# amoussawi/recoder

Hardware: AMD Instinct MI355X
Metric: train_users_per_sec (higher is better)
Workload: dtype f32 (decoder GEMMs: split 16-bit operands, f32 accumulate); 1 GPU; C2 ML-20M-like synthetic CSR 116677x20108 (lognormal degree mean 73, Zipf(1) items, values 1.0, seed 0); DynamicAutoencoder hidden=[200] tanh noise 0.5, MSE, dense Adam lr 1e-3 wd 2e-5, negative sampling; api=Recoder.train, batch_size_per_gpu=500, global_batch=500, parallelism=dp1, graph_replay=True, steps_per_graph=8, pretouch=parameters + Adam moments read 8 x in front of the clock (cache + clock warm)

## Files before the change

### recoder_amd/csrc/common.h

```cpp
#pragma once
#include <hip/hip_runtime.h>
#include <stdint.h>
#include <stdio.h>

#include "../../include/recoder_hip.h"
#include "../../include/recoder_hip_probe.h"
#include "internal.h"
int rk_tune_get(int knob);

void rk_set_error(const char *fmt, ...);

#define RK_LAUNCH(kernel, grid, block, shmem, stream, ...) \
  hipLaunchKernelGGL(kernel, grid, block, shmem, stream, __VA_ARGS__)

#define RK_CHECK_LAUNCH(name)                                              \
  do {                                                                     \
    hipError_t e__ = hipGetLastError();                                    \
    if (e__ != hipSuccess) {                                               \
      rk_set_error("%s: %s", name, hipGetErrorString(e__));                \
      return -1;                                                           \
    }                                                                      \
  } while (0)

#define RK_REQUIRE(cond, msg)                                              \
  do {                                                                     \
    if (!(cond)) {                                                         \
      rk_set_error("%s: %s", __func__, msg);                               \
      return -2;                                                           \
    }                                                                      \
  } while (0)

static inline int rk_cdiv(int64_t a, int64_t b) { return (int)((a + b - 1) / b); }

struct rk_enc_split_t;
int rk_ae_encode_fwd_at(const rk_block_t *blk, int32_t row_off, int32_t B, const float *W_en,
                        const float *b_en, int32_t h, const uint8_t *keep, float p, uint64_t seed,
                        const int64_t *cursor, int32_t cursor_off, const int64_t *users, int32_t act,
                        float *Z0, void *zt_planes, void *stream, const rk_enc_split_t *es,
                        uint64_t rng_step);
const rk_replay_t *rk_replay_get(void);
int rk_splitk_reduce(const float *ws, int M, int N, const int32_t *Kdev, int splits, const float *Zact,
                     int act, float *out, void *stream);
int rk_dz_splits(int B);
extern "C" int32_t rk_gemm_plain_bf16(void);
extern "C" int32_t rk_dw_pairs(void);
extern "C" int32_t rk_dw_encode_bwd_fused_ok(int32_t row_off, int32_t B);
int rk_adam_multi_at(const rk_adam_job_t *jobs, int32_t n_jobs, float *loss_part, int32_t n_part,
                     float denom, float *loss_out, const int64_t *cursor, int32_t cursor_off,
                     const void *table, int32_t tab_stride, const int32_t *tab_slots,
                     int64_t *cursor_next, int32_t advance, void *stream);

struct rk_small_gemm_t {
  const float *A; int lda, amode;
  const float *B; int ldb, bmode;
  int M, N, K;
  float *C; int ldc;
  const float *bias;
  int act, accumulate;
  const float *dact_y;
  int dact;
};
bool rk_small_gemm_fits(int M, int N, int K);
int rk_small_gemm(const rk_small_gemm_t *g, void *stream);
int rk_small_gemm_pair(const rk_small_gemm_t *g1, const rk_small_gemm_t *g2, void *stream);
int rk_small_gemm_pair_colsum(const rk_small_gemm_t *g1, const rk_small_gemm_t *g2, const float *cs_X,
                              int cs_rows, int cs_cols, float *cs_out, void *stream);
int rk_act_grad_colsum(float *dY, const float *Y, int rows, int cols, int act, float *db, void *stream);

__device__ __forceinline__ float rk_act(float x, int act) {
  switch (act) {
    case RK_ACT_TANH: return tanhf(x);
    case RK_ACT_SIGMOID: return 1.0f / (1.0f + expf(-x));
    case RK_ACT_RELU: return x > 0.f ? x : 0.f;
    case RK_ACT_SELU: {
      const float a = 1.6732632423543772848170429916717f;
      const float s = 1.0507009873554804934193349852946f;
      return s * (x > 0.f ? x : a * (expf(x) - 1.0f));
    }
    case RK_ACT_ELU: return x > 0.f ? x : (expf(x) - 1.0f);
    default: return x;
  }
}

__device__ __forceinline__ float rk_act_dy(float y, int act) {
  switch (act) {
    case RK_ACT_TANH: return 1.0f - y * y;
    case RK_ACT_SIGMOID: return (1.0f - y) * y;
    case RK_ACT_RELU: return y > 0.f ? 1.0f : 0.f;
    case RK_ACT_SELU: {
      const float a = 1.6732632423543772848170429916717f;
      const float s = 1.0507009873554804934193349852946f;
      return y > 0.f ? s : (y + s * a);
    }
    case RK_ACT_ELU: return y > 0.f ? 1.0f : (y + 1.0f);
    default: return 1.0f;
  }
}

__device__ __forceinline__ uint64_t rk_mix64(uint64_t z) {
  z = (z ^ (z >> 30)) * 0xbf58476d1ce4e5b9ULL;
  z = (z ^ (z >> 27)) * 0x94d049bb133111ebULL;
  return z ^ (z >> 31);
}
__device__ __forceinline__ bool rk_keep_draw(uint64_t seed, uint64_t step, uint64_t a,
                                             uint64_t b, float p) {
  uint64_t z = rk_mix64(seed + 0x9e3779b97f4a7c15ULL * (step + 1));
  z = rk_mix64(z ^ (a * 0xd1342543de82ef95ULL + b + 0x632be59bd9b4e019ULL));
  float u = (float)(z >> 40) * (1.0f / 16777216.0f);
  return u >= p;
}

struct rk_cur_t {
  const int64_t *cursor;
  int32_t off;
};
__device__ __forceinline__ int64_t rk_cur_global(const rk_cur_t &c) { return c.cursor[0] + c.off; }
__device__ __forceinline__ int64_t rk_cur_local(const rk_cur_t &c) {
  return c.cursor[0] - c.cursor[1] + c.off;
}
__device__ __forceinline__ int32_t rk_cur_stamp(const rk_cur_t &c) {
  return (int32_t)(rk_cur_global(c) & 0x3fffffff) + 1;
}

typedef __bf16 rk_bf16x2 __attribute__((ext_vector_type(2)));
typedef float rk_f32x2 __attribute__((ext_vector_type(2)));
__device__ __forceinline__ void rk_split_bf16_pair(float a, float b, uint32_t &h, uint32_t &m,
                                                   uint32_t &l) {
  const rk_f32x2 x = {a, b};
  const rk_bf16x2 hh = __builtin_convertvector(x, rk_bf16x2);
  const rk_f32x2 r1 = x - __builtin_convertvector(hh, rk_f32x2);
  const rk_bf16x2 mm = __builtin_convertvector(r1, rk_bf16x2);
  const rk_f32x2 r2 = r1 - __builtin_convertvector(mm, rk_f32x2);
  const rk_bf16x2 ll = __builtin_convertvector(r2, rk_bf16x2);
  h = __builtin_bit_cast(uint32_t, hh);
  m = __builtin_bit_cast(uint32_t, mm);
  l = __builtin_bit_cast(uint32_t, ll);
}

__device__ __forceinline__ float rk_wave_sum(float v) {
#pragma unroll
  for (int off = 32; off > 0; off >>= 1) v += __shfl_down(v, off, 64);
  return v;
}
__device__ __forceinline__ float rk_wave_max(float v) {
#pragma unroll
  for (int off = 32; off > 0; off >>= 1) v = fmaxf(v, __shfl_down(v, off, 64));
  return v;
}

__device__ __forceinline__ int rk_entry_index(const rk_block_t &b, int row, int c, uint32_t word) {
  return b.indptr[row] + b.pref_rc[(int64_t)row * b.ldw_rc + (c >> 5)] +
         __popc(word & ((1u << (c & 31)) - 1u));
}

__device__ __forceinline__ int rk_find_col(const int32_t *cols, int beg, int end, int c) {
  int lo = beg, hi = end;
  while (lo < hi) {
    int mid = (lo + hi) >> 1;
    if (cols[mid] < c) lo = mid + 1; else hi = mid;
  }
  return (lo < end && cols[lo] == c) ? lo : -1;
}
```

### recoder_amd/csrc/encoder.hip

```cpp
#include "common.h"
#include "encoder_bwd.h"
#include "planes.h"

namespace {

constexpr int FW = 8;
unsigned long long *g_enc_probe = nullptr;
#define ESTAMP(k) do { if (probe && threadIdx.x == 0) probe[(size_t)(blockIdx.x - n_split) * 8 + (k)] = wall_clock64(); } while (0)
template <int HV, int UB>
__global__ __launch_bounds__(FW * 64) void ae_encode_fwd_kernel(
    rk_block_t b, int row_off, int B, const float *__restrict__ W, const float *__restrict__ bias,
    int h, const uint8_t *__restrict__ keep, float p, float scale, uint64_t seed,
    uint64_t rng_step, const int64_t *__restrict__ users, const float *__restrict__ user_norm,
    int act, float *__restrict__ Z0, uint16_t *__restrict__ planes, int64_t plane_stride,
    int cols_pad, rk_cur_t cur, rkp::SplitW sw, int n_split, char *__restrict__ zimg, int z_kt,
    int zt_pairs, unsigned long long *probe, int z_ones) {
  __shared__ float red[FW];
  constexpr int PART_B = (FW - 1) * HV * 256 * 4;
  __shared__ __attribute__((aligned(16))) char sm_raw[PART_B > rkp::SPLIT_W_LDS ? PART_B : rkp::SPLIT_W_LDS];
  if ((int)blockIdx.x < n_split) {
    rkp::split_w_job<FW * 64>(sw, (int)blockIdx.x, sm_raw);
    return;
  }
  if (cur.cursor) {
    rng_step = (uint64_t)(rk_cur_global(cur) + 1);
    if (users) users += rk_cur_local(cur) * B;
  }
  float (*part)[HV * 256] = reinterpret_cast<float (*)[HV * 256]>(sm_raw);
  const int r = (int)blockIdx.x - n_split;
  if (r >= B) {
    if (planes) {
      for (int n = threadIdx.x; n < h; n += FW * 64) {
        const int64_t o = ((int64_t)(r >> 3) * cols_pad + n) * 8 + (r & 7);
        planes[o] = 0; planes[o + plane_stride] = 0; planes[o + 2 * plane_stride] = 0;
      }
    }
    return;
  }
  const int row = row_off + r;
  const int tid = threadIdx.x, lane = tid & 63, wid = tid >> 6;
  ESTAMP(0);
  const int beg = b.indptr[row], end = b.indptr[row + 1];
  const int n = end - beg;
  const bool implicit = b.implicit != 0;
  const int64_t uid = users ? users[row] : (int64_t)row;

  const int q = (n + FW - 1) / FW;
  const int wbeg = beg + wid * q;
  const int wend = min(end, wbeg + q);
  int item0 = 0;
  float v0 = 0.f;
  if (wbeg + lane < wend) {
    item0 = b.gcols ? b.gcols[wbeg + lane] : b.items[b.cols[wbeg + lane]];
    v0 = implicit ? 1.0f : b.vals[wbeg + lane];
  }

  float nrm;
  if (user_norm) {
    nrm = fmaxf(user_norm[uid], 1e-12f);
  } else if (implicit) {
    nrm = fmaxf(sqrtf((float)n), 1e-12f);
  } else {
    float ss = 0.f;
    for (int j = beg + tid; j < end; j += FW * 64) {
      const float v = b.vals[j];
      ss += v * v;
    }
    ss = rk_wave_sum(ss);
    if (lane == 0) red[wid] = ss;
    __syncthreads();
    float tot = 0.f;
#pragma unroll
    for (int w = 0; w < FW; ++w) tot += red[w];
    nrm = fmaxf(sqrtf(tot), 1e-12f);
  }

  if (probe) { if (item0 == 0x7fffffff && v0 == 1e30f) return; ESTAMP(1); }
  float4 acc[HV];
#pragma unroll
  for (int k = 0; k < HV; ++k) acc[k] = make_float4(0.f, 0.f, 0.f, 0.f);
  float4 bb[HV];
#pragma unroll
  for (int v = 0; v < HV; ++v) {
    const int hh = (v * 64 + lane) * 4;
    bb[v] = (bias && wid == 0 && hh < h) ? *reinterpret_cast<const float4 *>(bias + hh)
                                         : make_float4(0.f, 0.f, 0.f, 0.f);
  }

  for (int base = wbeg; base < wend; base += 64) {
    const int j = base + lane;
    int item = item0;
    float val = v0;
    if (base != wbeg && j < wend) {
      item = b.gcols ? b.gcols[j] : b.items[b.cols[j]];
      val = implicit ? 1.0f : b.vals[j];
    }
    float s = 0.f;
    if (j < wend) {
      const float xh = val / nrm;
      bool kp = true;
      if (p > 0.f) kp = keep ? (keep[j] != 0) : rk_keep_draw(seed, rng_step, (uint64_t)uid, (uint64_t)item, p);
      s = (p > 0.f) ? (kp ? xh * scale : 0.f) : xh;
      b.svals[j] = s;
    } else {
      item = 0;
    }
    unsigned long long live = __ballot(s != 0.f);
    while (live) {
      int it[UB];
      float sv[UB];
#pragma unroll
      for (int u = 0; u < UB; ++u) {
        const bool has = live != 0ull;
        const int kk = has ? __builtin_ctzll(live) : 0;
        live &= live - 1ull;
        it[u] = has ? __builtin_amdgcn_readlane(item, kk) : 0;
        sv[u] = has ? __int_as_float(__builtin_amdgcn_readlane(__float_as_int(s), kk)) : 0.f;
      }
#pragma unroll
      for (int v = 0; v < HV; ++v) {
        const int hh = min((v * 64 + lane) * 4, h - 4);
        float4 w4[UB];
#pragma unroll
        for (int u = 0; u < UB; ++u)
          w4[u] = *reinterpret_cast<const float4 *>(W + (int64_t)it[u] * h + hh);
#pragma unroll
        for (int u = 0; u < UB; ++u) {
          acc[v].x = fmaf(sv[u], w4[u].x, acc[v].x);
          acc[v].y = fmaf(sv[u], w4[u].y, acc[v].y);
          acc[v].z = fmaf(sv[u], w4[u].z, acc[v].z);
          acc[v].w = fmaf(sv[u], w4[u].w, acc[v].w);
        }
      }
    }
  }
  if (probe) { if (acc[0].x == 1.2345e30f) return; ESTAMP(2); }
  if (wid > 0) {
#pragma unroll
    for (int v = 0; v < HV; ++v)
      *reinterpret_cast<float4 *>(&part[wid - 1][(v * 64 + lane) * 4]) = acc[v];
  }
  __syncthreads();
  if (wid == 0) {
#pragma unroll
    for (int v = 0; v < HV; ++v) {
      const int hh = (v * 64 + lane) * 4;
      if (hh < h) {
        float4 a = acc[v];
        for (int w = 0; w < FW - 1; ++w) {
          const float4 o = *reinterpret_cast<const float4 *>(&part[w][hh]);
          a.x += o.x; a.y += o.y; a.z += o.z; a.w += o.w;
        }
        float4 y;
        y.x = rk_act(a.x + bb[v].x, act);
        y.y = rk_act(a.y + bb[v].y, act);
        y.z = rk_act(a.z + bb[v].z, act);
        y.w = rk_act(a.w + bb[v].w, act);
        *reinterpret_cast<float4 *>(Z0 + (int64_t)r * h + hh) = y;
        if (zimg) {
          const float sz = sw.plain ? 1.0f : rkp::SCALE_Z;
          rkp::store_split4(zimg + (int64_t)r * z_kt * rkp::LINE, hh, y, sz, sw.plain != 0);
          if (r == 0 && tid == 0) sw.scales[0] = sz;
          if ((h & 31) != 0 && hh == h - 4)
            rkp::store_split4(zimg + (int64_t)r * z_kt * rkp::LINE, h, make_float4(z_ones ? 1.f : 0.f, 0.f, 0.f, 0.f), sz,
                              sw.plain != 0);
        }
        if (planes) {
          uint32_t hp[2], mp[2], lp[2];
          if (zt_pairs) {
            uint2 hh2, ll2;
            rkp::split4(y, rkp::SCALE_Z, hh2, ll2);
            hp[0] = hh2.x; hp[1] = hh2.y; mp[0] = ll2.x; mp[1] = ll2.y; lp[0] = lp[1] = 0u;
          } else {
          rk_split_bf16_pair(y.x, y.y, hp[0], mp[0], lp[0]);
          rk_split_bf16_pair(y.z, y.w, hp[1], mp[1], lp[1]);
          }
#pragma unroll
          for (int e = 0; e < 4; ++e) {
            const int64_t o = ((int64_t)(r >> 3) * cols_pad + hh + e) * 8 + (r & 7);
            const int sh = (e & 1) * 16;
            planes[o] = (uint16_t)(hp[e >> 1] >> sh);
            planes[o + plane_stride] = (uint16_t)(mp[e >> 1] >> sh);
            planes[o + 2 * plane_stride] = (uint16_t)(lp[e >> 1] >> sh);
          }
        }
      }
    }
  }
  ESTAMP(3);
}

template <int HV>
__global__ __launch_bounds__(256) void ae_encode_bwd_kernel(
    rk_block_t b, int row_off, int B, const float *__restrict__ dZ, int h,
    float *__restrict__ G, int accumulate, float *__restrict__ gb, int n_gb) {
  ae_encode_bwd_body<HV>(b, row_off, B, dZ, h, G, accumulate, gb, n_gb, (int)blockIdx.x);
}

template <int HV, int WW>
__global__ __launch_bounds__(256) __attribute__((amdgpu_waves_per_eu(6))) void ae_encode_bwd_cols_light_kernel(
    rk_block_t b, int row_off, int B, const float *__restrict__ dZ, int h,
    float *__restrict__ G, int accumulate, float *__restrict__ gb, int n_gb) {
  ae_encode_bwd_cols_body<HV, false, WW, 2>(b, row_off, B, dZ, h, G, accumulate, gb, n_gb, (int)blockIdx.x);
}

template <int HV, int WW = 1, int U = 8>
__global__ __launch_bounds__(256) void ae_encode_bwd_cols_kernel(
    rk_block_t b, int row_off, int B, const float *__restrict__ dZ, int h,
    float *__restrict__ G, int accumulate, float *__restrict__ gb, int n_gb) {
  ae_encode_bwd_cols_body<HV, false, WW, U>(b, row_off, B, dZ, h, G, accumulate, gb, n_gb, (int)blockIdx.x);
}

}

static int encode_fwd_launch(const rk_block_t *blk, int32_t row_off, int32_t B, const float *W_en,
                             const float *b_en, int32_t h, const uint8_t *keep, float p,
                             uint64_t seed, uint64_t rng_step, const int64_t *users,
                             const float *user_norm, int32_t act, float *Z0, void *stream_,
                             void *zt_planes = nullptr, rk_cur_t cur = {nullptr, 0},
                             const rk_enc_split_t *es = nullptr, int zt_pairs = 0) {
  hipStream_t stream = (hipStream_t)stream_;
  RK_REQUIRE(h > 0 && h % 4 == 0 && h <= 1024, "h must be a multiple of 4, <= 1024");
  RK_REQUIRE(p >= 0.f && p < 1.f, "noise_prob must be in [0,1)");
  RK_REQUIRE(row_off >= 0 && B >= 0 && row_off + B <= blk->S_cap, "row slice out of range");
  RK_REQUIRE(user_norm == nullptr || users != nullptr, "user_norm is indexed by users[]");
  if (B == 0) return 0;
  const float scale = 1.0f / (float)(1.0 - (double)p);
  const int hv = rk_cdiv(h, 256);
  const int rows = zt_planes ? rk_dw3_rows_pad(B) : B;
  const int cols_pad = rk_dw3_cols_pad(h);
  const int64_t plane_stride = (int64_t)rk_dw3_rows_pad(B) * cols_pad;
  rkp::SplitW sw = {};
  int n_split = 0, z_kt = 0, z_ones = 0;
  char *zimg = nullptr;
  if (es) {
    sw = es->sw; n_split = es->n_split; zimg = es->zimg; z_kt = es->z_kt;
    z_ones = (es->z_ones && zimg && h % 32 != 0) ? 1 : 0;
  }
#define LAUNCH(HV)                                                                         \
  RK_LAUNCH((ae_encode_fwd_kernel<HV, 8>), dim3(n_split + rows), dim3(FW * 64), 0, stream, *blk, row_off, \
                     B, W_en, b_en, h, keep, p, scale, seed, rng_step, users, user_norm, act, Z0, \
                     (uint16_t *)zt_planes, plane_stride, cols_pad, cur, sw, n_split, zimg, z_kt, zt_pairs, g_enc_probe, z_ones)
  if (hv == 1) LAUNCH(1); else if (hv == 2) LAUNCH(2); else LAUNCH(4);
#undef LAUNCH
  RK_CHECK_LAUNCH("ae_encode_fwd");
  return 0;
}

extern "C" void rk_enc_probe(unsigned long long *buffer) { g_enc_probe = buffer; }

extern "C" int rk_ae_encode_fwd(const rk_block_t *blk, int32_t row_off, int32_t B,
                                const float *W_en, const float *b_en, int32_t h,
                                const uint8_t *keep, float p, uint64_t seed, uint64_t rng_step,
                                const int64_t *users, int32_t act, float *Z0, void *stream_) {
  RK_REQUIRE(b_en != nullptr, "b_en is required");
  if (const rk_replay_t *rp = rk_replay_get()) {
    const rk_cur_t cur = {rp->cursor, rp->off};
    return encode_fwd_launch(blk, row_off, B, W_en, b_en, h, keep, p, seed, 0, rp->users_base, nullptr,
                             act, Z0, stream_, nullptr, cur);
  }
  return encode_fwd_launch(blk, row_off, B, W_en, b_en, h, keep, p, seed, rng_step, users, nullptr,
                           act, Z0, stream_);
}

extern "C" int rk_ae_encode_fwd_split_w(const rk_block_t *blk, int32_t row_off, int32_t B,
                                        const float *W_en, const float *b_en, int32_t h,
                                        const uint8_t *keep, float p, uint64_t seed, uint64_t rng_step,
                                        const int64_t *users, int32_t act, float *Z0, const float *W_de,
                                        const int32_t *ranges, const rk_planes_t *pl, void *stream_) {
  RK_REQUIRE(b_en != nullptr, "b_en is required");
  RK_REQUIRE(pl && pl->h == h && blk->n_cap <= pl->n_cap, "planes were laid out for another shape");
  RK_REQUIRE((((uintptr_t)W_de) & 15) == 0, "W_de must be 16-byte aligned");
  rk_enc_split_t es = {};
  es.sw = rk_split_w_args(W_de, blk, ranges, pl);
  es.n_split = rk_cdiv(blk->n_cap, 32);
  es.zimg = nullptr;
  es.z_kt = rkp::kp_of(h) / 32;
  if (const rk_replay_t *rp = rk_replay_get()) {
    const rk_cur_t cur = {rp->cursor, rp->off};
    return encode_fwd_launch(blk, row_off, B, W_en, b_en, h, keep, p, seed, 0, rp->users_base, nullptr,
                             act, Z0, stream_, nullptr, cur, &es);
  }
  return encode_fwd_launch(blk, row_off, B, W_en, b_en, h, keep, p, seed, rng_step, users, nullptr,
                           act, Z0, stream_, nullptr, {nullptr, 0}, &es);
}

extern "C" int rk_ae_encode_fwd_planes(const rk_block_t *blk, int32_t row_off, int32_t B,
                                       const float *W_en, const float *b_en, int32_t h,
                                       const uint8_t *keep, float p, uint64_t seed, uint64_t rng_step,
                                       const int64_t *users, int32_t act, float *Z0, void *zt_planes,
                                       void *stream_) {
  RK_REQUIRE(b_en != nullptr, "b_en is required");
  RK_REQUIRE(zt_planes != nullptr && (((uintptr_t)zt_planes) & 15) == 0, "zt_planes: 16-byte aligned");
  return encode_fwd_launch(blk, row_off, B, W_en, b_en, h, keep, p, seed, rng_step, users, nullptr,
                           act, Z0, stream_, zt_planes);
}

int rk_ae_encode_fwd_at(const rk_block_t *blk, int32_t row_off, int32_t B, const float *W_en,
                        const float *b_en, int32_t h, const uint8_t *keep, float p, uint64_t seed,
                        const int64_t *cursor, int32_t cursor_off, const int64_t *users, int32_t act,
                        float *Z0, void *zt_planes, void *stream_, const rk_enc_split_t *es,
                        uint64_t rng_step) {
  const rk_cur_t cur = {cursor, cursor_off};
  return encode_fwd_launch(blk, row_off, B, W_en, b_en, h, keep, p, seed, rng_step, users, nullptr, act,
                           Z0, stream_, zt_planes, cur, es, zt_planes != nullptr && rk_dw_pairs() ? 1 : 0);
}

extern "C" int rk_ae_encode_fwd_partial(const rk_block_t *blk, int32_t row_off, int32_t B,
                                        const float *W_en, int32_t h, const uint8_t *keep, float p,
                                        uint64_t seed, uint64_t rng_step, const int64_t *users,
                                        const float *user_norm, float *Zpart, void *stream_) {
// ... 58 lines not shown
```

### recoder_amd/csrc/encoder_bwd.h

```cpp
#ifndef RK_ENCODER_BWD_H
#define RK_ENCODER_BWD_H
#include "common.h"

namespace {

template <int HV, bool DYN = false>
__device__ __forceinline__ void ae_encode_bwd_body(
    const rk_block_t &b, int row_off, int B, const float *__restrict__ dZ, int h,
    float *__restrict__ G, int accumulate, float *__restrict__ gb, int n_gb, int bid,
    int n_seg = 1, int64_t seg_stride = 0, char *sm = nullptr) {
  float (*part)[HV * 256];
  if constexpr (DYN) {
    part = reinterpret_cast<float (*)[HV * 256]>(sm);
  } else {
    __shared__ __attribute__((aligned(16))) float part_s[3][HV * 256];
    part = part_s;
  }
  const int lane = threadIdx.x & 63, wid = threadIdx.x >> 6;
  if (bid < n_gb) {
    const int gseg = bid % n_seg, j0 = (bid / n_seg) * 64 + (lane & 15) * 4;
    const int srows = ((B + n_seg - 1) / n_seg + 63) & ~63;
    const int r_lo = gseg * srows, r_hi = min(B, r_lo + srows);
    const int jj = min(j0, h - 4);
    float4 a = make_float4(0.f, 0.f, 0.f, 0.f);
    int r = r_lo + wid * 4 + (lane >> 4);
    for (; r + 7 * 16 < r_hi; r += 8 * 16) {
      float4 v[8];
#pragma unroll
      for (int u = 0; u < 8; ++u) v[u] = *reinterpret_cast<const float4 *>(dZ + (int64_t)(r + u * 16) * h + jj);
#pragma unroll
      for (int u = 0; u < 8; ++u) { a.x += v[u].x; a.y += v[u].y; a.z += v[u].z; a.w += v[u].w; }
    }
    for (; r < r_hi; r += 16) {
      const float4 v = *reinterpret_cast<const float4 *>(dZ + (int64_t)r * h + jj);
      a.x += v.x; a.y += v.y; a.z += v.z; a.w += v.w;
    }
#pragma unroll
    for (int off = 16; off <= 32; off <<= 1) {
      a.x += __shfl_xor(a.x, off, 64); a.y += __shfl_xor(a.y, off, 64);
      a.z += __shfl_xor(a.z, off, 64); a.w += __shfl_xor(a.w, off, 64);
    }
    if (lane < 16) *reinterpret_cast<float4 *>(&part[0][wid * 64 + lane * 4]) = a;
    __syncthreads();
    if (wid == 0 && lane < 16 && j0 < h) {
      float4 o = a;
      for (int w = 1; w < 4; ++w) {
        const float4 q = *reinterpret_cast<const float4 *>(&part[0][w * 64 + lane * 4]);
        o.x += q.x; o.y += q.y; o.z += q.z; o.w += q.w;
      }
      *reinterpret_cast<float4 *>(gb + gseg * h + j0) = o;
    }
    return;
  }
  const int n_b = b.counts[0];
  const int c = (bid - n_gb) / n_seg, seg = (bid - n_gb) % n_seg;
  if (c >= n_b) return;
  const uint32_t *colbits = b.bits_cr + (int64_t)c * b.ldw_cr;
  float4 acc[HV];
#pragma unroll
  for (int k = 0; k < HV; ++k) acc[k] = make_float4(0.f, 0.f, 0.f, 0.f);

  const int seg_rows = ((B + n_seg - 1) / n_seg + 63) & ~63;
  const int rbeg = row_off + seg * seg_rows;
  const int rend = min(row_off + B, rbeg + seg_rows);
  G += seg * seg_stride;
  for (int r0 = (rbeg & ~63) + wid * 64; r0 < rend; r0 += 256) {
    const int row = r0 + lane;
    bool on = false;
    float s = 0.f;
    if (row >= rbeg && row < rend) {
      on = (colbits[row >> 5] >> (row & 31)) & 1u;
      if (on) {
        const uint32_t word = b.bits_rc[(int64_t)row * b.ldw_rc + (c >> 5)];
        s = b.svals[rk_entry_index(b, row, c, word)];
      }
    }
    unsigned long long mask = __ballot(on && s != 0.f);
    while (mask) {
      int kk[8];
      float sv[8];
#pragma unroll
      for (int u = 0; u < 8; ++u) {
        const bool have = mask != 0ull;
        const int k = have ? __builtin_ctzll(mask) : 0;
        mask = have ? (mask & (mask - 1)) : 0ull;
        kk[u] = have ? (r0 + k - row_off) : 0;
        sv[u] = have ? __shfl(s, k, 64) : 0.f;
      }
#pragma unroll
      for (int v = 0; v < HV; ++v) {
        const int hh = min((v * 64 + lane) * 4, h - 4);
        float4 d4[8];
#pragma unroll
        for (int u = 0; u < 8; ++u)
          d4[u] = *reinterpret_cast<const float4 *>(dZ + (int64_t)kk[u] * h + hh);
#pragma unroll
        for (int u = 0; u < 8; ++u) {
          acc[v].x = fmaf(sv[u], d4[u].x, acc[v].x);
          acc[v].y = fmaf(sv[u], d4[u].y, acc[v].y);
          acc[v].z = fmaf(sv[u], d4[u].z, acc[v].z);
          acc[v].w = fmaf(sv[u], d4[u].w, acc[v].w);
        }
      }
    }
  }
  if (wid > 0) {
#pragma unroll
    for (int v = 0; v < HV; ++v)
      *reinterpret_cast<float4 *>(&part[wid - 1][(v * 64 + lane) * 4]) = acc[v];
  }
  __syncthreads();
  if (wid == 0) {
    float *grow = G + (int64_t)c * h;
#pragma unroll
    for (int v = 0; v < HV; ++v) {
      const int hh = (v * 64 + lane) * 4;
      if (hh < h) {
        float4 a = acc[v];
        for (int w = 0; w < 3; ++w) {
          const float4 o = *reinterpret_cast<const float4 *>(&part[w][hh]);
          a.x += o.x; a.y += o.y; a.z += o.z; a.w += o.w;
        }
        if (accumulate) {
          const float4 o = *reinterpret_cast<const float4 *>(grow + hh);
          a.x += o.x; a.y += o.y; a.z += o.z; a.w += o.w;
        }
        *reinterpret_cast<float4 *>(grow + hh) = a;
      }
    }
  }
}

template <int HV, bool DYN = false, int WW = 1, int U = 8>
__device__ __forceinline__ void ae_encode_bwd_cols_body(
    const rk_block_t &b, int row_off, int B, const float *__restrict__ dZ, int h,
    float *__restrict__ G, int accumulate, float *__restrict__ gb, int n_gb, const int bid,
    char *sm = nullptr) {
  static_assert(WW == 1 || !DYN, "the two-word window exists in the stand-alone kernel only");
  if (bid < n_gb) {
    ae_encode_bwd_body<HV, DYN>(b, row_off, B, dZ, h, G, accumulate, gb, n_gb, bid, 1, 0, sm);
    return;
  }
  float (*part)[HV * 256];
  uint16_t (*rows_l)[64];
  uint16_t *rows_h;
  int *heavy_l;
  if constexpr (DYN) {
    part = reinterpret_cast<float (*)[HV * 256]>(sm);
    rows_l = reinterpret_cast<uint16_t (*)[64]>(sm + 3 * HV * 256 * 4);
    rows_h = reinterpret_cast<uint16_t *>(sm + 3 * HV * 256 * 4 + 4 * 64 * 2);
    heavy_l = reinterpret_cast<int *>(sm + 3 * HV * 256 * 4 + 4 * 64 * 2 + (2048 + 64) * 2);
  } else {
    __shared__ __attribute__((aligned(16))) float part_s[3][HV * 256];
    __shared__ uint16_t rows_l_s[4][64];
    __shared__ uint16_t rows_h_s[WW * 2048 + 64];
    __shared__ int heavy_l_s[4];
    part = part_s; rows_l = rows_l_s; rows_h = rows_h_s; heavy_l = heavy_l_s;
  }
  const int lane = threadIdx.x & 63, wid = threadIdx.x >> 6;
  const int n_b = b.counts[0];
  const int Q = (n_b + 3) >> 2;
  const int c0 = bid - n_gb;
  if (c0 >= Q) return;
  const int c = c0 + wid * Q;
  const bool live = c < n_b;
  const int w0 = row_off >> 5, rend = row_off + B;
  const int nw = ((rend + 31) >> 5) - w0;
  uint32_t mw[WW];
  int off_w[WW];
  int total = 0;
#pragma unroll
  for (int j = 0; j < WW; ++j) {
    const int wj = lane + 64 * j;
    uint32_t m = 0;
    if (live && wj < nw) {
      m = b.bits_cr[(int64_t)c * b.ldw_cr + w0 + wj];
      const int base = (w0 + wj) << 5;
      if (base < row_off) m &= ~0u << (row_off - base);
      if (base + 32 > rend) m &= (1u << (rend - base)) - 1u;
    }
    mw[j] = m;
  }
#pragma unroll
  for (int j = 0; j < WW; ++j) {
    const int cnt = __popc(mw[j]);
    int incl = cnt;
#pragma unroll
    for (int d = 1; d < 64; d <<= 1) {
      const int t = __shfl_up(incl, d, 64);
      if (lane >= d) incl += t;
    }
    off_w[j] = total + incl - cnt;
    total += __shfl(incl, 63, 64);
  }
  const bool heavy = total > 64;
  if (lane == 0) heavy_l[wid] = heavy ? total : 0;
  if (!heavy) {
#pragma unroll
    for (int j = 0; j < WW; ++j) {
      uint32_t m = mw[j];
      int o = off_w[j];
      while (m) {
        const int k = __builtin_ctz(m);
        m &= m - 1;
        rows_l[wid][o++] = (uint16_t)(((w0 + lane + 64 * j) << 5) + k - row_off);
      }
    }
  }
  __syncthreads();
  float4 acc[HV];
#pragma unroll
  for (int k = 0; k < HV; ++k) acc[k] = make_float4(0.f, 0.f, 0.f, 0.f);
  if (live && !heavy && total > 0) {
    int row = row_off;
    float sv = 0.f;
    if (lane < total) {
      row = row_off + rows_l[wid][lane];
      const uint32_t word = b.bits_rc[(int64_t)row * b.ldw_rc + (c >> 5)];
      sv = b.svals[rk_entry_index(b, row, c, word)];
    }
    unsigned long long lv = __ballot(sv != 0.f);
    while (lv) {
      int kk[U];
      float s8[U];
#pragma unroll
      for (int u = 0; u < U; ++u) {
        const bool has = lv != 0ull;
        const int k = has ? __builtin_ctzll(lv) : 0;
        lv &= lv - 1ull;
        kk[u] = has ? __builtin_amdgcn_readlane(row, k) - row_off : 0;
        s8[u] = has ? __int_as_float(__builtin_amdgcn_readlane(__float_as_int(sv), k)) : 0.f;
      }
#pragma unroll
      for (int v = 0; v < HV; ++v) {
        const int hh = min((v * 64 + lane) * 4, h - 4);
        float4 d4[U];
#pragma unroll
        for (int u = 0; u < U; ++u)
          d4[u] = *reinterpret_cast<const float4 *>(dZ + (int64_t)kk[u] * h + hh);
#pragma unroll
        for (int u = 0; u < U; ++u) {
          acc[v].x = fmaf(s8[u], d4[u].x, acc[v].x);
          acc[v].y = fmaf(s8[u], d4[u].y, acc[v].y);
          acc[v].z = fmaf(s8[u], d4[u].z, acc[v].z);
          acc[v].w = fmaf(s8[u], d4[u].w, acc[v].w);
        }
      }
    }
  }
  if (live && !heavy && !(accumulate && total == 0)) {
    float *grow = G + (int64_t)c * h;
#pragma unroll
    for (int v = 0; v < HV; ++v) {
      const int hh = (v * 64 + lane) * 4;
      if (hh < h) {
        float4 a = acc[v];
        if (accumulate) {
          const float4 o = *reinterpret_cast<const float4 *>(grow + hh);
          a.x += o.x; a.y += o.y; a.z += o.z; a.w += o.w;
        }
        *reinterpret_cast<float4 *>(grow + hh) = a;
      }
    }
  }
  for (int j = 0; j < 4; ++j) {
    const int tot_j = heavy_l[j];
    if (tot_j == 0) continue;
    const int cj = c0 + j * Q;
    if (wid == j) {
#pragma unroll
      for (int jw = 0; jw < WW; ++jw) {
        uint32_t m = mw[jw];
        int o = off_w[jw];
        while (m) {
          const int k = __builtin_ctz(m);
          m &= m - 1;
          rows_h[o++] = (uint16_t)(((w0 + lane + 64 * jw) << 5) + k - row_off);
        }
      }
    }
    __syncthreads();
#pragma unroll
    for (int k = 0; k < HV; ++k) acc[k] = make_float4(0.f, 0.f, 0.f, 0.f);
    const int per = (tot_j + 3) >> 2;
    const int e1 = min(tot_j, (wid + 1) * per);
    for (int e0 = wid * per; e0 < e1; e0 += 64) {
      const int ne = min(64, e1 - e0);
      int row = row_off;
      float sv = 0.f;
      if (lane < ne) {
        row = row_off + rows_h[e0 + lane];
        const uint32_t word = b.bits_rc[(int64_t)row * b.ldw_rc + (cj >> 5)];
        sv = b.svals[rk_entry_index(b, row, cj, word)];
      }
      constexpr int UH = U >= 8 ? 16 : 2 * U;
      unsigned long long lv = __ballot(sv != 0.f);
      while (lv) {
        int kk[UH];
        float s16[UH];
#pragma unroll
        for (int u = 0; u < UH; ++u) {
          const bool has = lv != 0ull;
          const int k = has ? __builtin_ctzll(lv) : 0;
          lv &= lv - 1ull;
          kk[u] = has ? __builtin_amdgcn_readlane(row, k) - row_off : 0;
          s16[u] = has ? __int_as_float(__builtin_amdgcn_readlane(__float_as_int(sv), k)) : 0.f;
        }
#pragma unroll
        for (int v = 0; v < HV; ++v) {
          const int hh = min((v * 64 + lane) * 4, h - 4);
          float4 d4[UH];
#pragma unroll
          for (int u = 0; u < UH; ++u)
            d4[u] = *reinterpret_cast<const float4 *>(dZ + (int64_t)kk[u] * h + hh);
#pragma unroll
          for (int u = 0; u < UH; ++u) {
            acc[v].x = fmaf(s16[u], d4[u].x, acc[v].x);
            acc[v].y = fmaf(s16[u], d4[u].y, acc[v].y);
            acc[v].z = fmaf(s16[u], d4[u].z, acc[v].z);
            acc[v].w = fmaf(s16[u], d4[u].w, acc[v].w);
          }
        }
      }
    }
    if (wid > 0) {
#pragma unroll
      for (int v = 0; v < HV; ++v)
        *reinterpret_cast<float4 *>(&part[wid - 1][(v * 64 + lane) * 4]) = acc[v];
    }
    __syncthreads();
    if (wid == 0) {
      float *grow = G + (int64_t)cj * h;
#pragma unroll
      for (int v = 0; v < HV; ++v) {
        const int hh = (v * 64 + lane) * 4;
        if (hh < h) {
          float4 a = acc[v];
          for (int w = 0; w < 3; ++w) {
            const float4 o = *reinterpret_cast<const float4 *>(&part[w][hh]);
            a.x += o.x; a.y += o.y; a.z += o.z; a.w += o.w;
          }
          if (accumulate) {
            const float4 o = *reinterpret_cast<const float4 *>(grow + hh);
            a.x += o.x; a.y += o.y; a.z += o.z; a.w += o.w;
          }
          *reinterpret_cast<float4 *>(grow + hh) = a;
        }
      }
    }
    __syncthreads();
  }
}

}
#endif
```

### recoder_amd/csrc/fdecode.hip

```cpp
#include <stdlib.h>

#include <algorithm>

#include <type_traits>

#include "common.h"
#include "pgemm_epi.h"
#include "planes.h"

namespace {

using pg::f16x8;
using pg::f32x16;

struct FdecP {
  const char *zimg, *wimg;
  const float *scales;
  int KT;
  int M;
  const int32_t *Ndev;
  int z_rows, w_rows;
  rk_block_t blk;
  int row_off;
  float confidence, inv_B;
// ... 61 lines not shown
    words[i] = b.bits_rc[(int64_t)mrow * b.ldw_rc + min((n0 >> 5) + 2 * hf + i, b.ldw_rc - 1)];
  if (tid < 128) misc[tid] = p.bias[p.bidx[min(n0 + tid, N - 1)]];

  pg::Opnd ow = {p.wimg, (int64_t)KT * 128, KT, p.w_rows};
  pg::Stager<128, false, 8> sw;
  sw.init(ow, n0, 0, min(N, p.w_rows), wave, lane);
#pragma unroll
  for (int kt = 0; kt < KTM; ++kt) sw.issue(Wst + kt * WB, wave);
  asm volatile("" ::: "memory");
  pg::u32x4 zraw[KTM][4];
  {
    const int zlim = min(M, p.z_rows) - 1;
#pragma unroll
    for (int i = 0; i < 4; ++i) {
      const int zr = min(m0 + 32 * pr + 8 * i + (lane >> 3), zlim);
      const char *zsrc = p.zimg + (int64_t)zr * (KTM * 128) + 16 * (lane & 7);
#pragma unroll
      for (int kt = 0; kt < KTM; ++kt) zraw[kt][i] = *reinterpret_cast<const pg::u32x4 *>(zsrc + kt * 128);
    }
  }
  asm volatile("s_waitcnt vmcnt(%0) lgkmcnt(0)" ::"n"(4 * KTM) : "memory");
  __builtin_amdgcn_s_barrier();
  asm volatile("" ::: "memory");

  f32x16 acc[2];
#pragma unroll
  for (int i = 0; i < 2; ++i)
#pragma unroll
    for (int r = 0; r < 16; ++r) acc[i][r] = 0.f;
  pg::FragKC fr;
  fr.init(lane);
  char *zb = Zb + wave * 4096;
#pragma unroll
  for (int kt = 0; kt < KTM; ++kt) {
    const char *SW = Wst + kt * WB + hf * 8192;
    __builtin_amdgcn_wave_barrier();
#pragma unroll
    for (int i = 0; i < 4; ++i) {
      const int r = 8 * i + (lane >> 3);
      *reinterpret_cast<pg::u32x4 *>(zb + r * 128 + (((lane & 7) ^ pg::kc_sw(r)) << 4)) = zraw[kt][i];
    }
    __builtin_amdgcn_fence(__ATOMIC_RELEASE, "wavefront");
    __builtin_amdgcn_wave_barrier();
    __builtin_amdgcn_fence(__ATOMIC_ACQUIRE, "wavefront");
    f16x8 zh[2], zl[2];
#pragma unroll
    for (int ks = 0; ks < 2; ++ks) { zh[ks] = fr.load(zb, 0, ks, 0); if (!PLAIN) zl[ks] = fr.load(zb, 0, ks, 1); }
#pragma unroll
    for (int ks = 0; ks < 2; ++ks) {
      f16x8 wh[2], wl[2];
#pragma unroll
      for (int i = 0; i < 2; ++i) { wh[i] = fr.load(SW, i, ks, 0); if (!PLAIN) wl[i] = fr.load(SW, i, ks, 1); }
      if constexpr (PLAIN) {
#pragma unroll
        for (int i = 0; i < 2; ++i)
          acc[i] = __builtin_amdgcn_mfma_f32_32x32x16_bf16(__builtin_bit_cast(pg::bf16x8, wh[i]),
                                                           __builtin_bit_cast(pg::bf16x8, zh[ks]), acc[i], 0, 0, 0);
        continue;
      }
#pragma unroll
      for (int i = 0; i < 2; ++i) acc[i] = __builtin_amdgcn_mfma_f32_32x32x16_f16(wh[i], zl[ks], acc[i], 0, 0, 0);
#pragma unroll
      for (int i = 0; i < 2; ++i) acc[i] = __builtin_amdgcn_mfma_f32_32x32x16_f16(wl[i], zh[ks], acc[i], 0, 0, 0);
#pragma unroll
      for (int i = 0; i < 2; ++i) acc[i] = __builtin_amdgcn_mfma_f32_32x32x16_f16(wh[i], zh[ks], acc[i], 0, 0, 0);
    }
  }

  const float inv = 1.0f / (p.scales[0] * p.scales[1]);
  const bool implicit = b.implicit != 0;
  const int nh = n0 + 64 * hf;
  float lsum = 0.f, gmax = 0.f;
  auto loss_pass = [&](auto implicit_c) {
    constexpr bool IMPL = decltype(implicit_c)::value;
#pragma unroll
    for (int i = 0; i < 2; ++i) {
      const uint32_t w = words[i];
#pragma unroll
      for (int r = 0; r < 16; ++r) {
        const int nl = (r & 3) + 8 * (r >> 2) + 4 * lh;
        const int n = nh + 32 * i + nl;
        const bool ok = (m < M) && (n < N);
        const float o = acc[i][r] * inv + misc[64 * hf + 32 * i + nl];
        float tv = 0.f;
        if (ok && ((w >> nl) & 1u)) {
          tv = 1.0f;
          if (!IMPL) tv = b.vals[rk_entry_index(b, mrow, n, w)];
        }
        float l, g;
        if (LOSS == pg::LOSS_MSE) {
          const float wgt = (tv > 0.f) ? (1.0f + p.confidence) : 1.0f;
          const float d = o - tv;
          l = wgt * (d * d);
          g = (2.0f * d) * (wgt * p.inv_B);
        } else {
          const float ls = fminf(o, 0.f) - log1pf(expf(-fabsf(o)));
          l = (1.0f - tv) * o - ls;
          const float sg = 1.0f / (1.0f + expf(-o));
          g = (sg - tv) * p.inv_B;
        }
        if (ok) { lsum += l; gmax = fmaxf(gmax, fabsf(g)); } else g = 0.f;
        acc[i][r] = g;
      }
    }
  };
  auto loss_pass_mse_implicit = [&]() {
    const float c = p.confidence, inv_B2 = 2.0f * p.inv_B;
#pragma unroll
    for (int i = 0; i < 2; ++i) {
      const int nrem = N - (nh + 32 * i);
      uint32_t vmask = nrem >= 32 ? 0xffffffffu : (nrem <= 0 ? 0u : ((1u << nrem) - 1u));
      if (m >= M) vmask = 0u;
      const uint32_t vsh = vmask >> (4 * lh), wsh = (words[i] & vmask) >> (4 * lh);
#pragma unroll
      for (int q = 0; q < 4; ++q) {
        const float4 bq = *reinterpret_cast<const float4 *>(misc + 64 * hf + 32 * i + 8 * q + 4 * lh);
        const float bias4[4] = {bq.x, bq.y, bq.z, bq.w};
#pragma unroll
        for (int e = 0; e < 4; ++e) {
          const int r = 4 * q + e, bp = e + 8 * q;
          const float bitf = (float)((wsh >> bp) & 1u);
          const uint32_t okm = (uint32_t)(((int32_t)(vsh << (31 - bp))) >> 31);
          const float o = acc[i][r] * inv + bias4[e];
          const float d = o - bitf;
          const float w = fmaf(c, bitf, 1.0f);
          const float l = w * (d * d);
          lsum += __uint_as_float(__float_as_uint(l) & okm);
          const float g = __uint_as_float(__float_as_uint(d * (w * inv_B2)) & okm);
          gmax = fmaxf(gmax, fabsf(g));
          acc[i][r] = g;
        }
      }
    }
  };
  if (implicit && LOSS == pg::LOSS_MSE) loss_pass_mse_implicit();
  else if (implicit) loss_pass(std::true_type{});
  else loss_pass(std::false_type{});
#pragma unroll
  for (int off = 32; off > 0; off >>= 1) gmax = fmaxf(gmax, __shfl_xor(gmax, off, 64));
  lsum = rk_wave_sum(lsum);
  float s_do = 1.0f;
  if (!PLAIN && gmax > 0.f) {
    const int ex = min(max((int)(__float_as_uint(gmax) >> 23) - 127, -100), 100);
    s_do = __uint_as_float((uint32_t)(13 - ex + 127) << 23);
  }
  if (lane == 0) {
    misc[128 + wave] = lsum;
    misc[136 + wave] = gmax;
    if ((m0 >> 5) + pr < ((M + 31) >> 5) && 2 * nt + hf < p.ds_pitch)
      p.dscale[(int64_t)((m0 >> 5) + pr) * p.ds_pitch + 2 * nt + hf] = s_do;
  }

  const int ldi = b.counts[2];
  char *drow = p.dimg + (int64_t)m * ldi * 4 + (int64_t)(nh >> 5) * 128;
  const bool st_ok = m < p.rows_img;
  f32x16 acc2[KTM];
#pragma unroll
  for (int j = 0; j < KTM; ++j)
#pragma unroll
    for (int r = 0; r < 16; ++r) acc2[j][r] = 0.f;
#pragma unroll
  for (int i = 0; i < 2; ++i) {
#pragma unroll
    for (int s = 0; s < 2; ++s) {
      uint2 fh, fl, sh, sl;
      if constexpr (PLAIN) {
        rkp::plain4(make_float4(acc[i][8 * s + 0], acc[i][8 * s + 1], acc[i][8 * s + 2], acc[i][8 * s + 3]), fh, fl);
        rkp::plain4(make_float4(acc[i][8 * s + 4], acc[i][8 * s + 5], acc[i][8 * s + 6], acc[i][8 * s + 7]), sh, sl);
      } else {
      rkp::split4(make_float4(acc[i][8 * s + 0], acc[i][8 * s + 1], acc[i][8 * s + 2], acc[i][8 * s + 3]), s_do, fh, fl);
      rkp::split4(make_float4(acc[i][8 * s + 4], acc[i][8 * s + 5], acc[i][8 * s + 6], acc[i][8 * s + 7]), s_do, sh, sl);
      }
      swap32(fh.x, sh.x); swap32(fh.y, sh.y); swap32(fl.x, sl.x); swap32(fl.y, sl.y);
      const uint4 hi4 = make_uint4(fh.x, fh.y, sh.x, sh.y), lo4 = make_uint4(fl.x, fl.y, sl.x, sl.y);
      if (st_ok && nh + 32 * i < ldi) {
        char *d = drow + i * 128 + (16 * s + 8 * lh) * 2;
        *reinterpret_cast<uint4 *>(d) = hi4;
        *reinterpret_cast<uint4 *>(d + 64) = lo4;
      }
      const f16x8 dh = __builtin_bit_cast(f16x8, hi4), dl = __builtin_bit_cast(f16x8, lo4);
      const int row0 = 64 * hf + 32 * i + 16 * s + 8 * lh;
#pragma unroll
      for (int j = 0; j < KTM; ++j) {
        if constexpr (PLAIN) {
          const f16x8 ah = w_tr_frag(Wst + j * WB, row0, lane, 0);
          acc2[j] = __builtin_amdgcn_mfma_f32_32x32x16_bf16(__builtin_bit_cast(pg::bf16x8, ah), __builtin_bit_cast(pg::bf16x8, dh),
                                                            acc2[j], 0, 0, 0);
        } else {
          const f16x8 ah = w_tr_frag(Wst + j * WB, row0, lane, 0), al = w_tr_frag(Wst + j * WB, row0, lane, 1);
          acc2[j] = __builtin_amdgcn_mfma_f32_32x32x16_f16(al, dh, acc2[j], 0, 0, 0);
          acc2[j] = __builtin_amdgcn_mfma_f32_32x32x16_f16(ah, dl, acc2[j], 0, 0, 0);
          acc2[j] = __builtin_amdgcn_mfma_f32_32x32x16_f16(ah, dh, acc2[j], 0, 0, 0);
        }
      }
    }
  }
  constexpr int PITCH = FD_PITCH(KTM);
  float *X = reinterpret_cast<float *>(smem) + pr * 32 * PITCH;
  const float inv2 = 1.0f / (s_do * p.scales[1]);
  __syncthreads();
  if (hf == 1) {
#pragma unroll
    for (int j = 0; j < KTM; ++j)
#pragma unroll
      for (int q = 0; q < 4; ++q)
        *reinterpret_cast<float4 *>(X + l31 * PITCH + 32 * j + 8 * q + 4 * lh) =
            make_float4(acc2[j][4 * q] * inv2, acc2[j][4 * q + 1] * inv2, acc2[j][4 * q + 2] * inv2, acc2[j][4 * q + 3] * inv2);
  }
  __syncthreads();
  if (hf == 0) {
#pragma unroll
    for (int j = 0; j < KTM; ++j)
#pragma unroll
      for (int q = 0; q < 4; ++q) {
        float4 *x = reinterpret_cast<float4 *>(X + l31 * PITCH + 32 * j + 8 * q + 4 * lh);
        const float4 u = *x;
        *x = make_float4(acc2[j][4 * q] * inv2 + u.x, acc2[j][4 * q + 1] * inv2 + u.y, acc2[j][4 * q + 2] * inv2 + u.z,
                         acc2[j][4 * q + 3] * inv2 + u.w);
      }
  }
  __syncthreads();
  {
    const int h4 = p.h >> 2;
    const int rows = min(32, M - (m0 + 32 * pr));
    float4 *ws = reinterpret_cast<float4 *>(p.dz_ws + ((int64_t)nt * M + m0 + 32 * pr) * p.h);
    for (int idx = hf * 64 + lane; idx < rows * h4; idx += 128) {
      const int row = idx / h4, c = idx - row * h4;
      ws[idx] = *reinterpret_cast<const float4 *>(X + row * PITCH + 4 * c);
    }
  }
  if (tid == 0) {
    float ls = 0.f, gm = 0.f;
#pragma unroll
    for (int w = 0; w < 8; ++w) { ls += misc[128 + w]; gm = fmaxf(gm, misc[136 + w]); }
    p.loss_part[t] = ls;
    atomicMax(reinterpret_cast<unsigned int *>(b.counts) + 8 + ((int)blockIdx.x & 63), __float_as_uint(gm));
  }
}

inline bool al16(const void *q) { return ((uintptr_t)q & 15) == 0; }

}

int rk_fdec_slabs(int B, int n_cap) {
  (void)B;
  return rk_cdiv(n_cap, 128);
}

extern "C" int rk_fdec_dz_reduce(const float *dz_workspace, int32_t B, int32_t h, const rk_block_t *tgt,
                                 const float *Zact, int32_t act, float *dZ, void *stream_) {
  RK_REQUIRE(al16(dz_workspace) && al16(dZ), "operands must be 16-byte aligned");
  if (B == 0) return 0;
  return rk_splitk_reduce_tiles(dz_workspace, B, h, tgt->counts, rk_fdec_slabs(B, tgt->n_cap), 128, Zact, act, dZ,
                                stream_);
}

extern "C" int32_t rk_fdec_ok(int32_t B, int32_t h, int32_t n_cap, int32_t loss_kind) {
  static const int on = [] { const char *e = getenv("RK_FDEC"); return (e && atoi(e) == 0) ? 0 : 1; }();
  const int kt = rkp::kp_of(h) / 32;
  return on && rk_pg_enabled() && rk_gemm_split16() &&
         (loss_kind == RK_LOSS_MSE || loss_kind == RK_LOSS_BCE) && h % 4 == 0 && h <= 224 &&
         B < 1024 &&
         (kt == 2 || kt == 4 || kt == 7) &&
         (int64_t)rk_fdec_slabs(B, n_cap) * B * h * (int64_t)sizeof(float) <= ((int64_t)4 << 30) ? 1 : 0;
}
extern "C" int64_t rk_fdec_workspace_bytes(int32_t B, int32_t h, int32_t n_cap) {
  int64_t rows = 0;
  for (int b = 1; b <= B; ++b) rows = std::max(rows, (int64_t)rk_fdec_slabs(b, n_cap) * b);
  return rows * h * (int64_t)sizeof(float);
}

extern "C" int rk_fdec_loss_dz(const rk_planes_t *pl, int32_t B, const rk_block_t *tgt, int32_t row_off,
                               const float *b_de, int32_t loss_kind, float confidence, float inv_B,
                               void *dO_img, int32_t rows_img, float *dO_scales, float *loss_part,
                               float *dz_workspace, void *stream_) {
  hipStream_t stream = (hipStream_t)stream_;
  RK_REQUIRE(pl && B <= pl->B_cap && tgt->n_cap <= pl->n_cap, "planes were laid out for another shape");
  RK_REQUIRE(row_off >= 0 && row_off + B <= tgt->S_cap, "row slice out of range");
  RK_REQUIRE(rk_fdec_ok(B, pl->h, tgt->n_cap, loss_kind), "shape / loss outside the fused decode (rk_fdec_ok)");
  RK_REQUIRE(tgt->implicit || tgt->pref_rc != nullptr, "explicit values need pref_rc");
  RK_REQUIRE(dO_img && dO_scales && al16(dO_img) && al16(dz_workspace) && rows_img >= ((B + 31) & ~31),
             "dO image: 16-byte aligned, round_up(B, 32) rows; a scale table");
  if (B == 0) return 0;
  FdecP p = {};
  p.zimg = (const char *)pl->z; p.wimg = (const char *)pl->w; p.scales = pl->scales;
  p.KT = rkp::kp_of(pl->h) / 32;
  p.M = B; p.Ndev = tgt->counts; p.z_rows = pl->B_cap; p.w_rows = pl->n_cap;
  p.blk = *tgt; p.row_off = row_off; p.confidence = confidence; p.inv_B = inv_B;
  p.bias = b_de; p.bidx = tgt->items; p.loss_part = loss_part;
  p.dimg = (char *)dO_img; p.rows_img = rows_img; p.dscale = dO_scales; p.ds_pitch = rk_cdiv(tgt->n_cap, 64);
  p.dz_ws = dz_workspace; p.h = pl->h;
  const int grid = rk_cdiv(rk_cdiv(B, 128) * rk_cdiv(tgt->n_cap, 128), 8) * 8;
  const bool plain = rk_gemm_plain_bf16() != 0;
#define GO(KTM, LOSS)                                                                                          \
  do {                                                                                                         \
    if (plain) {                                                                                               \
      auto k = fdec_kernel<KTM, LOSS, true>;                                                                   \
      static const hipError_t attr = hipFuncSetAttribute((const void *)k, hipFuncAttributeMaxDynamicSharedMemorySize, 160 * 1024); \
      if (attr != hipSuccess) { rk_set_error("LDS attribute"); return -1; }                                    \
      hipLaunchKernelGGL(k, dim3(grid), dim3(512), FD_LDS(KTM), stream, p);                                    \
    } else {                                                                                                   \
      auto k = fdec_kernel<KTM, LOSS>;                                                                         \
      static const hipError_t attr = hipFuncSetAttribute((const void *)k, hipFuncAttributeMaxDynamicSharedMemorySize, 160 * 1024); \
      if (attr != hipSuccess) { rk_set_error("LDS attribute"); return -1; }                                    \
      hipLaunchKernelGGL(k, dim3(grid), dim3(512), FD_LDS(KTM), stream, p);                                    \
    }                                                                                                          \
  } while (0)
#define BY_KT(LOSS)                                                                                            \
  do { if (p.KT == 2) GO(2, LOSS); else if (p.KT == 4) GO(4, LOSS); else GO(7, LOSS); } while (0)
  if (loss_kind == RK_LOSS_MSE) BY_KT(pg::LOSS_MSE); else BY_KT(pg::LOSS_BCE);
#undef BY_KT
#undef GO
  RK_CHECK_LAUNCH("fdec_loss_dz");
  return 0;
}
```

### recoder_amd/csrc/splitk_reduce.h

```cpp
#pragma once
#include "common.h"

namespace rkred {

constexpr int RED_W = 8;
struct Args {
  const float *ws;
  int M, N;
  const int32_t *Kdev;
  int tile_k, max_splits;
  const float *Zact;
  int act;
  float *out;
};
inline int blocks(int M, int N) { return (int)(((int64_t)M * N / 4 + 63) / 64); }

template <int RW = RED_W>
__device__ __forceinline__ void body(const Args &a, const int block, float4 (*part)[64]) {
  const int K = *a.Kdev;
  const int kchunk = a.tile_k > 0 ? a.tile_k : ((K + a.max_splits - 1) / a.max_splits + 31) & ~31;
  int ns = (K + kchunk - 1) / kchunk;
  if (ns > a.max_splits) ns = a.max_splits;
  const int64_t tot4 = ((int64_t)a.M * a.N) >> 2;
  const float4 *ws4 = reinterpret_cast<const float4 *>(a.ws);
  const int lane = threadIdx.x & 63, q = threadIdx.x >> 6;
  const int64_t i = (int64_t)block * 64 + lane;
  const int per = (ns + RW - 1) / RW;
  const int z1 = min(ns, (q + 1) * per);
  float4 s = make_float4(0.f, 0.f, 0.f, 0.f);
  float4 y = make_float4(0.f, 0.f, 0.f, 0.f);
  if (a.Zact && q == 0 && i < tot4) y = reinterpret_cast<const float4 *>(a.Zact)[i];
  if (i < tot4) {
    int z = q * per;
    for (; z + 8 <= z1; z += 8) {
      float4 v[8];
#pragma unroll
      for (int u = 0; u < 8; ++u) v[u] = ws4[(int64_t)(z + u) * tot4 + i];
#pragma unroll
      for (int u = 0; u < 8; ++u) { s.x += v[u].x; s.y += v[u].y; s.z += v[u].z; s.w += v[u].w; }
    }
    for (; z < z1; ++z) {
      const float4 v = ws4[(int64_t)z * tot4 + i];
      s.x += v.x; s.y += v.y; s.z += v.z; s.w += v.w;
    }
  }
  if (q > 0) part[q - 1][lane] = s;
  __syncthreads();
  if (q == 0 && i < tot4) {
#pragma unroll
    for (int w = 0; w < RW - 1; ++w) {
      const float4 b = part[w][lane];
      s.x += b.x; s.y += b.y; s.z += b.z; s.w += b.w;
    }
    if (a.Zact) {
      s.x *= rk_act_dy(y.x, a.act); s.y *= rk_act_dy(y.y, a.act);
      s.z *= rk_act_dy(y.z, a.act); s.w *= rk_act_dy(y.w, a.act);
    }
    reinterpret_cast<float4 *>(a.out)[i] = s;
  }
}

}
```

Before: 4.358 million users/s.

## Use sc1 cache-policy stores for intermediates and stage fdecode image rows through LDS

Adds a rk_store16 helper that emits global_store_dwordx4 with the sc1 cache-policy bit, selectable per call site through compile-time macros. It is applied to the encoder Z output, the encoder backward gradient rows, the fdecode dz slab, and the split-k reduce output, so these intermediates are written under a different cache policy before the next kernel reads them. In fdecode, the split image tiles are now written into swizzled LDS first and then read back as full 128-byte lines, so each global store is contiguous rather than scattered. The cost is extra LDS traffic, wave barriers and inline asm with a hand-placed s_nop, whose effect on caching and correctness depends on the hardware.

```diff
diff --git a/recoder_amd/csrc/common.h b/recoder_amd/csrc/common.h
--- a/recoder_amd/csrc/common.h
+++ b/recoder_amd/csrc/common.h
@@ -137,6 +137,39 @@
   l = __builtin_bit_cast(uint32_t, ll);
 }
 
+#ifndef RK_WT_FDEC_IMG
+#define RK_WT_FDEC_IMG 1
+#endif
+#ifndef RK_WT_FDEC_SLAB
+#define RK_WT_FDEC_SLAB 1
+#endif
+#ifndef RK_WT_REDUCE
+#define RK_WT_REDUCE 1
+#endif
+#ifndef RK_WT_ENC_BWD
+#define RK_WT_ENC_BWD 1
+#endif
+#ifndef RK_WT_ENC_Z
+#define RK_WT_ENC_Z 1
+#endif
+typedef uint32_t rk_u32x4 __attribute__((ext_vector_type(4)));
+template <bool WT>
+__device__ __forceinline__ void rk_store16(void *p, const rk_u32x4 v) {
+  if constexpr (WT) {
+    asm volatile("global_store_dwordx4 %0, %1, off sc1\n\ts_nop 1" ::"v"(p), "v"(v) : "memory");
+  } else {
+    *reinterpret_cast<rk_u32x4 *>(p) = v;
+  }
+}
+template <bool WT>
+__device__ __forceinline__ void rk_store16(void *p, const float4 v) {
+  rk_store16<WT>(p, rk_u32x4{__float_as_uint(v.x), __float_as_uint(v.y), __float_as_uint(v.z), __float_as_uint(v.w)});
+}
+template <bool WT>
+__device__ __forceinline__ void rk_store16(void *p, const uint4 v) {
+  rk_store16<WT>(p, rk_u32x4{v.x, v.y, v.z, v.w});
+}
+
 __device__ __forceinline__ float rk_wave_sum(float v) {
 #pragma unroll
   for (int off = 32; off > 0; off >>= 1) v += __shfl_down(v, off, 64);
diff --git a/recoder_amd/csrc/encoder.hip b/recoder_amd/csrc/encoder.hip
--- a/recoder_amd/csrc/encoder.hip
+++ b/recoder_amd/csrc/encoder.hip
@@ -156,7 +156,7 @@
         y.y = rk_act(a.y + bb[v].y, act);
         y.z = rk_act(a.z + bb[v].z, act);
         y.w = rk_act(a.w + bb[v].w, act);
-        *reinterpret_cast<float4 *>(Z0 + (int64_t)r * h + hh) = y;
+        rk_store16<RK_WT_ENC_Z != 0>(Z0 + (int64_t)r * h + hh, y);
         if (zimg) {
           const float sz = sw.plain ? 1.0f : rkp::SCALE_Z;
           rkp::store_split4(zimg + (int64_t)r * z_kt * rkp::LINE, hh, y, sz, sw.plain != 0);
diff --git a/recoder_amd/csrc/encoder_bwd.h b/recoder_amd/csrc/encoder_bwd.h
--- a/recoder_amd/csrc/encoder_bwd.h
+++ b/recoder_amd/csrc/encoder_bwd.h
@@ -125,7 +125,7 @@
           const float4 o = *reinterpret_cast<const float4 *>(grow + hh);
           a.x += o.x; a.y += o.y; a.z += o.z; a.w += o.w;
         }
-        *reinterpret_cast<float4 *>(grow + hh) = a;
+        rk_store16<RK_WT_ENC_BWD != 0>(grow + hh, a);
       }
     }
   }
@@ -259,7 +259,7 @@
           const float4 o = *reinterpret_cast<const float4 *>(grow + hh);
           a.x += o.x; a.y += o.y; a.z += o.z; a.w += o.w;
         }
-        *reinterpret_cast<float4 *>(grow + hh) = a;
+        rk_store16<RK_WT_ENC_BWD != 0>(grow + hh, a);
       }
     }
   }
@@ -344,7 +344,7 @@
             const float4 o = *reinterpret_cast<const float4 *>(grow + hh);
             a.x += o.x; a.y += o.y; a.z += o.z; a.w += o.w;
           }
-          *reinterpret_cast<float4 *>(grow + hh) = a;
+          rk_store16<RK_WT_ENC_BWD != 0>(grow + hh, a);
         }
       }
     }
diff --git a/recoder_amd/csrc/fdecode.hip b/recoder_amd/csrc/fdecode.hip
--- a/recoder_amd/csrc/fdecode.hip
+++ b/recoder_amd/csrc/fdecode.hip
@@ -237,8 +237,9 @@
   }
 
   const int ldi = b.counts[2];
-  char *drow = p.dimg + (int64_t)m * ldi * 4 + (int64_t)(nh >> 5) * 128;
-  const bool st_ok = m < p.rows_img;
+  const int mr0 = m0 + 32 * pr + (lane >> 3);
+  char *drow = p.dimg + (int64_t)mr0 * ldi * 4 + (int64_t)(nh >> 5) * 128 + 16 * (lane & 7);
+  char *zwr = zb + fr.base;
   f32x16 acc2[KTM];
 #pragma unroll
   for (int j = 0; j < KTM; ++j)
@@ -258,11 +259,9 @@
       }
       swap32(fh.x, sh.x); swap32(fh.y, sh.y); swap32(fl.x, sl.x); swap32(fl.y, sl.y);
       const uint4 hi4 = make_uint4(fh.x, fh.y, sh.x, sh.y), lo4 = make_uint4(fl.x, fl.y, sl.x, sl.y);
-      if (st_ok && nh + 32 * i < ldi) {
-        char *d = drow + i * 128 + (16 * s + 8 * lh) * 2;
-        *reinterpret_cast<uint4 *>(d) = hi4;
-        *reinterpret_cast<uint4 *>(d + 64) = lo4;
-      }
+      if (s == 0) __builtin_amdgcn_wave_barrier();
+      *reinterpret_cast<uint4 *>(zwr + (((2 * s + lh) ^ fr.sw) << 4)) = hi4;
+      *reinterpret_cast<uint4 *>(zwr + (((4 + 2 * s + lh) ^ fr.sw) << 4)) = lo4;
       const f16x8 dh = __builtin_bit_cast(f16x8, hi4), dl = __builtin_bit_cast(f16x8, lo4);
       const int row0 = 64 * hf + 32 * i + 16 * s + 8 * lh;
 #pragma unroll
@@ -279,6 +278,20 @@
         }
       }
     }
+    __builtin_amdgcn_fence(__ATOMIC_RELEASE, "wavefront");
+    __builtin_amdgcn_wave_barrier();
+    __builtin_amdgcn_fence(__ATOMIC_ACQUIRE, "wavefront");
+    if (nh + 32 * i < ldi) {
+      pg::u32x4 line[4];
+#pragma unroll
+      for (int k = 0; k < 4; ++k) {
+        const int r = 8 * k + (lane >> 3);
+        line[k] = *reinterpret_cast<const pg::u32x4 *>(zb + r * 128 + (((lane & 7) ^ pg::kc_sw(r)) << 4));
+      }
+#pragma unroll
+      for (int k = 0; k < 4; ++k)
+        if (mr0 + 8 * k < p.rows_img) rk_store16<RK_WT_FDEC_IMG != 0>(drow + (int64_t)(8 * k) * ldi * 4 + i * 128, line[k]);
+    }
   }
   constexpr int PITCH = FD_PITCH(KTM);
   float *X = reinterpret_cast<float *>(smem) + pr * 32 * PITCH;
@@ -311,7 +324,7 @@
     float4 *ws = reinterpret_cast<float4 *>(p.dz_ws + ((int64_t)nt * M + m0 + 32 * pr) * p.h);
     for (int idx = hf * 64 + lane; idx < rows * h4; idx += 128) {
       const int row = idx / h4, c = idx - row * h4;
-      ws[idx] = *reinterpret_cast<const float4 *>(X + row * PITCH + 4 * c);
+      rk_store16<RK_WT_FDEC_SLAB != 0>(ws + idx, *reinterpret_cast<const float4 *>(X + row * PITCH + 4 * c));
     }
   }
   if (tid == 0) {
diff --git a/recoder_amd/csrc/splitk_reduce.h b/recoder_amd/csrc/splitk_reduce.h
--- a/recoder_amd/csrc/splitk_reduce.h
+++ b/recoder_amd/csrc/splitk_reduce.h
@@ -56,7 +56,7 @@
       s.x *= rk_act_dy(y.x, a.act); s.y *= rk_act_dy(y.y, a.act);
       s.z *= rk_act_dy(y.z, a.act); s.w *= rk_act_dy(y.w, a.act);
     }
-    reinterpret_cast<float4 *>(a.out)[i] = s;
+    rk_store16<RK_WT_REDUCE != 0>(reinterpret_cast<float4 *>(a.out) + i, s);
   }
 }
 
```

Result: no change. 4.338 million users/s (median of 2 runs) (-0.5%).
